# Kostis-S-Z/exploring_meta

Measured on AMD Instinct MI355X. Metric: tasks/sec, higher is better.
Workload: dtype f32

## Files before the change

### exploring_meta_amd/csrc/conv_b16.h

```cpp
#pragma once

#ifndef MI_CONV_B16_DEFAULT
#define MI_CONV_B16_DEFAULT 1
#endif

__device__ __forceinline__ void buf_st2_untracked(mi_u32x4 rsrc, unsigned off, float v0, float v1) {
  floatx2 v = {v0, v1};
  asm volatile("buffer_store_dwordx2 %0, %1, %2, 0 offen" : : "v"(v), "v"(off), "s"(rsrc) : "memory");
}
__device__ __forceinline__ floatx2 buf_ld8(mi_rsrc r, unsigned off) {
  return __builtin_bit_cast(floatx2, __builtin_amdgcn_raw_buffer_load_b64(r, off, 0, 0));
}
__device__ __forceinline__ int lane_mask_bit_rt(unsigned v, int bit) {
  int r;
  asm("v_bfe_i32 %0, %1, %2, 1" : "=v"(r) : "v"(v), "i"(bit));
  return r;
}
__device__ __forceinline__ float bf16_sub_v(float a, float b) {
  float r;
  asm volatile("v_sub_f32 %0, %1, %2" : "=v"(r) : "v"(a), "v"(b));
  return r;
}
#define MI_B16_MFMA(x, y, acc) __builtin_amdgcn_mfma_f32_16x16x32_bf16(MI_BF8(x), MI_BF8(y), acc, 0, 0, 0)

// ... 41 lines not shown
  {
    const unsigned total = gridDim.x * gridDim.y * gridDim.z;
    if ((total & 7u) == 0u) {
      const unsigned lin = (blockIdx.z * gridDim.y + blockIdx.y) * gridDim.x + blockIdx.x;
      const unsigned nl = (lin & 7u) * (total >> 3) + (lin >> 3);
      ct = (int)(nl % gridDim.z);
      bx = (int)((nl / gridDim.z) % gridDim.x);
      task = (int)(nl / (gridDim.z * gridDim.x));
    }
  }
  const int H = a.g.h, W = a.g.w;
  const int cbase = ct * 32;
  B16_ST(unsigned long long* stp = (blockIdx.x == 0 && blockIdx.y == 0 && blockIdx.z == 0 && (wave & 3) == 0 && lane == 0 && g_conv_stamps) ? g_conv_stamps + (wave >> 2) * 8 : nullptr;
         unsigned long long st_k = 0, st_epi = 0, st_n = 0, st_a = 0, st_b = 0, st_comb = 0; if (stp) stp[0] = __builtin_amdgcn_s_memtime();)

  {
    mi_u32x4* lw = reinterpret_cast<mi_u32x4*>(lds);
    constexpr int NIT = NU * 2 * 64, IPT = (NIT + NT - 1) / NT;
    floatx4 w0[IPT], w1[IPT];
#pragma unroll
    for (int q = 0; q < IPT; ++q) {
      const int it = tid + q * NT;
      const int ln = it & 63, grp = it >> 6;
      const int nb = grp & 1, u = grp >> 1;
      const int cc = u % NCC, tt = u / NCC, term = tt / 9, tap = tt - term * 9;
      const int k0 = cc * 32 + (ln >> 4) * 8, co = cbase + 2 * (ln & 15) + nb;
      const bool live = it < NIT;
      const float* wsrc = a.wt[live ? term : 0] + (size_t)task * a.wstride;
      if (MODE == 0) {
        const float* src = wsrc + ((size_t)(live ? tap : 0) * CI + k0) * CO + co;
#pragma unroll
// ... 379 lines not shown
```

### exploring_meta_amd/csrc/conv_mfma.hip

```cpp
#include "mi_common.h"
#include "kernels.h"
#include "bf16_split.h"
#include "fold.h"
#include <type_traits>

#ifdef MI_CONV_ABLATE_LOW
#define MI_LOW_PRODUCT(X)
#else
#define MI_LOW_PRODUCT(X) X
#endif
#ifdef MI_CONV_ABLATE_ROW
#define MI_ROW_KEPT(i) (hg_ddy(i) != 1)
#else
#define MI_ROW_KEPT(i) true
#endif
#define EPI_NONE 0
#define EPI_STATS 1
#define EPI_TSTATS 2
#define EPI_BRED 3

__device__ __forceinline__ void stats_block_reduce(double s, double q, double* ldsd, int lane, int wave, int nwaves,
                                                   double* partial_task, int co_total, int cbase, const FinArgs& fin, int task,
                                                   int bx = -1) {
  double* partial_blk = partial_task + (size_t)(bx < 0 ? (int)blockIdx.x : bx) * 2 * co_total;
// ... 233 lines not shown
  const int cbase = ct * 32;
  unsigned long long* cstamp = (blockIdx.x == 0 && blockIdx.y == 0 && blockIdx.z == 0) ? g_conv_stamps : nullptr;
  CV_STAMP(0);

  constexpr int NQ = BF ? 0 : NTERMS * 9 * CI * 32 / 4;
  float f16_sa[NTERMS], f16_sw[NTERMS], f16_inv = 1.f;
#pragma unroll
  for (int t = 0; t < NTERMS; ++t) { f16_sa[t] = 1.f; f16_sw[t] = 1.f; }
  unsigned f16_amax[NTERMS];
#pragma unroll
  for (int t = 0; t < NTERMS; ++t) f16_amax[t] = 0u;
  if constexpr (F16) {
#pragma unroll
    for (int t = 0; t < NTERMS; ++t) f16_amax[t] = mi_cell_fetch(a.amax[t], task);
  }
  if constexpr (BF) {
    mi_u32x4* l4 = reinterpret_cast<mi_u32x4*>(lds);
    constexpr int NIT = NSTEP * 2 * 64, IPT = (NIT + NT - 1) / NT;
    floatx4 w0[IPT], w1[IPT];
#pragma unroll
    for (int q = 0; q < IPT; ++q) {
      const int it = tid + q * NT;
      const int ln = it & 63, grp = it >> 6;
      const int jj = ln & 31, hb = ln >> 5, kb = grp & 1, stp = grp >> 1;
      const int cc = stp % NCC, tt = stp / NCC, term = tt / 9, tap = tt - term * 9;
      const int k0 = cc * 32 + hb * 16 + kb * 8;
      const bool live = it < NIT;
      const float* wsrc = a.wt[live ? term : 0] + (size_t)task * a.wstride;
      if (MODE == 0) {
        const float* src = wsrc + ((size_t)(live ? tap : 0) * CI + k0) * CO + cbase + jj;
#pragma unroll
// ... 850 lines not shown
    if (a.split_bf16) return launch_conv_s1_bf<CI, NTERMS, EPI, MODE, false>(st, a, grid);
  }
  const size_t lds = (size_t)NTERMS * 9 * CI * 32 * sizeof(float);
  auto k = conv3x3_s1_mfma_kernel<CI, NTERMS, EPI, MODE>;
  static unsigned attr_done = 0;
  if (hipError_t e = ensure_dynamic_lds(reinterpret_cast<const void*>(k), lds, &attr_done); e != hipSuccess) return e;
  hipLaunchKernelGGL(k, grid, dim3(ConvWaves<CI, NTERMS>::value * 64), lds, st, a);
  return hipGetLastError();
}

static bool conv_s1_ok(const ConvArgs& a) {
  return a.g.stride == 1 && a.g.co == a.g.ci && a.g.h == a.g.ho && a.g.w == a.g.wo && a.mpix < (1 << 24) &&
         (size_t)a.mpix * a.g.ci * 4 < (size_t)MI_OOB;
}

template <int CI, int NTERMS, int EPI>
static hipError_t launch_conv_ms(hipStream_t st, ConvArgs& a, dim3 grid, int mode, int stride) {
  if constexpr (EPI == EPI_BRED) {
    if (conv_s1_ok(a) && mode == 1) return launch_conv_s1<CI, NTERMS, EPI_BRED, 1>(st, a, grid);
    return hipErrorInvalidValue;
  } else {
    if (conv_s1_ok(a)) {
      if (mode == 0) return launch_conv_s1<CI, NTERMS, EPI, 0>(st, a, grid);
      if (EPI == EPI_NONE && mode == 1) return launch_conv_s1<CI, NTERMS, EPI_NONE, 1>(st, a, grid);
      return hipErrorInvalidValue;
    }
    if (mode == 0 && stride == 1) return launch_conv_t<CI, NTERMS, EPI, 0, 1>(st, a, grid);
    if (mode == 0 && stride == 2) return launch_conv_t<CI, NTERMS, EPI, 0, 2>(st, a, grid);
    if (EPI == EPI_NONE) {
      if (mode == 1 && stride == 1) return launch_conv_t<CI, NTERMS, EPI_NONE, 1, 1>(st, a, grid);
// ... 3 lines not shown
  }
}

hipError_t launch_conv3x3(hipStream_t st, ConvArgs a, int tasks, int nterms, int epi, int mode, int* blocks_per_task) {
  const int cot = a.g.co / 32;
  int ntiles, tpw;
  dim3 grid;
  a.split_bf16 = ((a.g.ci == 32 || (a.g.ci == 64 && nterms == 1)) && conv_s1_ok(a) && conv_split_bf16() &&
                  (epi == EPI_BRED ? mode == 1 : (mode == 0 || epi == EPI_NONE)) &&
                  ((g_conv_split_mask >> (((nterms - 1) * 2 + mode) * 4 + epi)) & 1u)) ? conv_operand_form() : 0;
  if (a.split_bf16 == 2 && (!a.amax[0] || (nterms == 2 && !a.amax[1]))) a.split_bf16 = 1;
  const int nw = ((a.split_bf16 == 2 && MI_F16_WIDE) || (nterms == 2 && a.g.ci == 32) || (a.split_bf16 && a.g.ci == 64)) ? 8 : 4;
  conv_grid(a.mpix, tasks, cot, nw, a.g.ci, nterms, ntiles, tpw, grid, a.split_bf16 ? 30 : 32, a.split_bf16 == 2 && MI_F16_WIDE && epi != EPI_TSTATS);
  a.ntiles = ntiles;
  a.tiles_per_wave = tpw;
  a.stagger = conv_stagger();
  if (blocks_per_task) *blocks_per_task = grid.x;
  if (a.g.co % 32 != 0) return hipErrorInvalidValue;
  const int s = a.g.stride;
  if (a.g.ci == 1 || a.g.ci == 3) {
    if (mode != 0 || nterms != 1) return hipErrorInvalidValue;
#define FIRST(CI0, E, S) hipLaunchKernelGGL((conv3x3_first_mfma_kernel<CI0, E, S>), grid, dim3(256), 0, st, a)
    if (a.g.ci == 3 && s == 1) { if (epi == EPI_STATS) FIRST(3, EPI_STATS, 1); else if (epi == EPI_TSTATS) FIRST(3, EPI_TSTATS, 1); else FIRST(3, EPI_NONE, 1); }
    else if (a.g.ci == 3 && s == 2) { if (epi == EPI_STATS) FIRST(3, EPI_STATS, 2); else if (epi == EPI_TSTATS) FIRST(3, EPI_TSTATS, 2); else FIRST(3, EPI_NONE, 2); }
    else if (a.g.ci == 1 && s == 1) { if (epi == EPI_STATS) FIRST(1, EPI_STATS, 1); else if (epi == EPI_TSTATS) FIRST(1, EPI_TSTATS, 1); else FIRST(1, EPI_NONE, 1); }
    else if (a.g.ci == 1 && s == 2) { if (epi == EPI_STATS) FIRST(1, EPI_STATS, 2); else if (epi == EPI_TSTATS) FIRST(1, EPI_TSTATS, 2); else FIRST(1, EPI_NONE, 2); }
    else return hipErrorInvalidValue;
#undef FIRST
    return hipGetLastError();
  }
// ... 1 lines not shown
  if (nterms == 1) {                                                                              \
    if (epi == EPI_NONE) return launch_conv_ms<CI, 1, EPI_NONE>(st, a, grid, mode, s);             \
    if (epi == EPI_STATS) return launch_conv_ms<CI, 1, EPI_STATS>(st, a, grid, mode, s);           \
    if (epi == EPI_BRED) return launch_conv_ms<CI, 1, EPI_BRED>(st, a, grid, mode, s);             \
    return launch_conv_ms<CI, 1, EPI_TSTATS>(st, a, grid, mode, s);                                \
  } else {                                                                                        \
    if (epi == EPI_NONE) return launch_conv_ms<CI, 2, EPI_NONE>(st, a, grid, mode, s);             \
    if (epi == EPI_TSTATS) return launch_conv_ms<CI, 2, EPI_TSTATS>(st, a, grid, mode, s);         \
    if (epi == EPI_BRED) return launch_conv_ms<CI, 2, EPI_BRED>(st, a, grid, mode, s);             \
    return hipErrorInvalidValue;                                                                  \
  }
  if (a.g.ci == 32) { DISPATCH(32) }
  if (a.g.ci == 64) { DISPATCH(64) }
#undef DISPATCH
  return hipErrorInvalidValue;
}

int wgrad_chunks(int mpix, int tasks) {
  int chunk = 1024;
  while (chunk > 32 && (long)ceil_div(mpix, chunk) * tasks < 2048) chunk >>= 1;
  return chunk;
}

static int rows_pick_rh(int w) {
  const int cand[4] = {7, 8, 5, 4};
  int best = 7, best_waste = 1 << 30;
  for (int i = 0; i < 4; ++i) {
    const int waste = ceil_div(w, cand[i]) * cand[i] - w;
    if (waste < best_waste) { best_waste = waste; best = cand[i]; }
  }
// ... 167 lines not shown
```

### exploring_meta_amd/csrc/engine.hip

```cpp
#include <string>
#include <vector>
#include <cstdio>
#include <cmath>
#include <cstring>
#include "mi_common.h"
#include "kernels.h"
#include "../../include/mi_maml.h"

#define EPI_NONE 0
#define EPI_STATS 1
#define EPI_TSTATS 2
#define EPI_BRED 3

static thread_local std::string g_err;

struct Layer {
  int ci, co, h, w, ho, wo, stride, pool, hp, wp;
  size_t off_gamma, off_beta, off_w, off_b;
};

static int gram_query_env() { static const int v = getenv("MI_GRAM_QUERY") ? atoi(getenv("MI_GRAM_QUERY")) : 2; return v; }
static bool fork_once_env() { static const bool v = getenv("MI_FORK_ONCE") && atoi(getenv("MI_FORK_ONCE")) != 0; return v; }
struct mi_engine {
  mi_model_desc d;
// ... 317 lines not shown
  float *xs, *xq;
  int32_t *ys, *yq;
  std::vector<ActSet> sup;
  ActSet qry;
  TanSet tan;
  double* bnpart;
  float* wgpart;
  float* wgpart_side;
  float* wgpart_l[8];
  double *gram_part, *gram_s;
  double *gram_q, *gram_part_q;
  int half = 0;
  float *tmp_loss, *tmp_acc;
  float* hscr;
  float* tail_wpart = nullptr; double* tail_bpart = nullptr; float* tail_scr = nullptr;
  unsigned* cells;
  int cell_cap, cell_used = 0, cell_T = 0;
  bool f16 = false;
  std::vector<std::pair<const void*, unsigned*>> cellmap;
  size_t bytes;
};

static void plan_actset(const mi_engine* e, Bump& b, ActSet& A, int T, int n, bool with_bwd) {
  const int nl = (int)e->L.size();
  A.zhm = nullptr;
  A.arg0 = nullptr;
  for (int l = 0; l < 8; ++l) A.zhl[l] = nullptr;
  for (int l = 0; l < nl; ++l) {
    const Layer& L = e->L[l];
    const size_t zs = (size_t)T * n * L.ho * L.wo * L.co, ps = (size_t)T * n * L.hp * L.wp * L.co;
// ... 4 lines not shown
    A.dp[l] = with_bwd ? b.take<float>(ps) : nullptr;
    if (fused && with_bwd && e->gram1) { A.zhm = b.take<float>(ps); A.arg0 = b.take<uint8_t>(ps); }
    A.zhl[l] = (!fused && with_bwd && l >= 1 && L.pool && dgrad_carries_reduce(e, l + 1)) ? b.take<float>(ps) : nullptr;
    A.mu[l] = b.take<float>((size_t)T * L.co);
    A.rstd[l] = b.take<float>((size_t)T * L.co);
  }
  if (e->d.head_mean_pool) {
    A.f = b.take<float>((size_t)T * n * e->feat);
    A.df = with_bwd ? b.take<float>((size_t)T * n * e->feat) : nullptr;
  } else {
    A.f = A.p[nl - 1];
    A.df = A.dp[nl - 1];
  }
  A.prob = b.take<float>((size_t)T * n * e->d.ways);
  A.dl = b.take<float>((size_t)T * n * e->d.ways);
}

static unsigned long long kernel_selection_key() {
  unsigned mask = 0;
  const unsigned form = (unsigned)mi_conv_get_split_bf16(&mask);
  return (unsigned long long)form + 4ull * (unsigned)conv_b16() + 16ull * (unsigned)block1_split_form() + 64ull * (unsigned)sparse_wgrad_split_form() + 128ull * (unsigned long long)mask;
}

static void make_plan(const mi_engine* e, void* ws, int T, int ns, int nq, int K, int second_order, Plan& pl) {
  Bump b{reinterpret_cast<char*>(ws), 0};
  const int nl = (int)e->L.size();
  const size_t TP = (size_t)T * e->PS;
  pl.theta = b.take<float>(TP * (K + 1));
  pl.g = b.take<float>(TP * (K > 0 ? K : 1));
  pl.lam = b.take<float>(TP);
// ... 72 lines not shown
      X.rdz[l] = (l == 0 && e->fuse1) ? nullptr : b.take<float>((size_t)T * ns * L.ho * L.wo * L.co);
    }
    X.dpd[0] = b.take<float>(pmax);
    X.dpd[1] = b.take<float>(pmax);
    if (e->d.head_mean_pool) {
      X.fd = b.take<float>((size_t)T * ns * e->feat);
      X.rdf = b.take<float>((size_t)T * ns * e->feat);
    } else {
      X.fd = nullptr;
      X.rdf = nullptr;
    }
  }
  pl.cell_cap = 8 + (K + 1) * 2 * nl + K * 4 * nl + 4 * nl;
  pl.cells = conv_operand_form() == 2 ? b.take<unsigned>((size_t)pl.cell_cap * T * MI_CELL_WORDS) : nullptr;
  pl.cell_T = T;
  pl.bytes = align_up(b.off, 256);
}

static int plan_begin(mi_engine* e, hipStream_t st, Plan& pl) {
  pl.f16 = conv_operand_form() == 2;
  pl.cell_used = 0;
  pl.cellmap.clear();
  if (pl.f16) HIPCHK(e, hipMemsetAsync(pl.cells, 0, (size_t)pl.cell_cap * pl.cell_T * MI_CELL_WORDS * sizeof(unsigned), st));
  return MI_OK;
}
static unsigned* cell_bind(mi_engine* e, Plan& pl, const void* tensor) {
  static const bool no_hooks = getenv("MI_F16_NO_PRODUCER_AMAX") && atoi(getenv("MI_F16_NO_PRODUCER_AMAX")) != 0;
  if (!pl.f16 || !tensor) return nullptr;
  for (auto it = pl.cellmap.begin(); it != pl.cellmap.end(); ++it)
    if (it->first == tensor) { pl.cellmap.erase(it); break; }
  if (no_hooks || pl.cell_used >= pl.cell_cap) return nullptr;
// ... 61 lines not shown
      !pl.tail_wpart)
    return false;
  const Layer& L = e->L[nl - 1];
  return tail_supported(n, L.ho, L.wo, L.co, L.pool, e->feat, e->d.ways);
}
static void tail_common(const mi_engine* e, const Plan& pl, TailArgs& ta) {
  ta.wpart = pl.tail_wpart; ta.bpart = pl.tail_bpart; ta.scr = pl.tail_scr; ta.counter = e->counters; ta.stamps = e->tail_stamps;
}
extern "C" int mi_debug_tail_stamps(mi_engine* e, unsigned long long* buf) {
  if (!e) return MI_ERR_ARG;
  e->tail_stamps = buf;
  return MI_OK;
}

static int trunk_forward(mi_engine* e, hipStream_t st, Plan& pl, ActSet& A, const float* x0, int n, int T, const float* theta,
                         const double* gram = nullptr, bool stats_ready = false, bool skip_last_bn = false) {
  const int nl = (int)e->L.size();
  const size_t P = e->PS;
  for (int l = 0; l < nl; ++l) {
    const Layer& L = e->L[l];
    if (l == 0 && e->fuse1) {
      B1Args ba = b1_args(e, pl, A, x0, n, theta);
      int blk = 0;
      if (gram && stats_ready) {
      } else if (gram) {
        LAUNCH(e, st, OP_GRAM_STATS, 0, launch_gram_stats(st, gram, T, L.ci, L.co, theta + L.off_w, P, nullptr, 0, 1.0 / ((double)n * L.ho * L.wo), 0, A.mu[0], A.rstd[0], nullptr, nullptr));
      } else {
        ba.fin = fin_of(e, T, 1.0 / ((double)n * L.ho * L.wo), FIN_STATS, A.mu[0], L.co, A.rstd[0], L.co);
        LAUNCH(e, st, OP_CONV_FWD, 0, launch_block1(st, ba, T, L.ci, B1_STATS, &blk));
        if (!ba.fin.counter)
          LAUNCH(e, st, OP_BN_FINALIZE, 0, launch_bn_finalize(st, pl.bnpart, blk, T, L.co, 1.0 / ((double)n * L.ho * L.wo), FIN_STATS, A.mu[0], L.co, A.rstd[0], L.co));
        ba.fin = FinArgs{};
      }
// ... 4 lines not shown
      ba.fwd_fp32 = (gram && A.arg0) ? 0 : 1;
      LAUNCH(e, st, OP_BN_FWD, 0, launch_block1(st, ba, T, L.ci, B1_FWD, nullptr));
      continue;
    }
    ConvArgs ca{};
    ca.in[0] = l == 0 ? x0 : A.p[l - 1];
    ca.wt[0] = theta + L.off_w;
    ca.wstride = P;
    ca.out = A.z[l];
    ca.partial = pl.bnpart;
    ca.g = geom(L, n);
    ca.mpix = n * L.ho * L.wo;
    int blk = 0;
    ca.fin = fin_of(e, T, 1.0 / (double)ca.mpix, FIN_STATS, A.mu[l], L.co, A.rstd[l], L.co);
    if (l >= 1) CELL(ca.in[0], (size_t)n * L.h * L.w * L.ci, ca.amax[0]);
    LAUNCH(e, st, OP_CONV_FWD, l, launch_conv3x3(st, ca, T, 1, EPI_STATS, 0, &blk));
    if (!ca.fin.counter)
      LAUNCH(e, st, OP_BN_FINALIZE, l, launch_bn_finalize(st, pl.bnpart, blk, T, L.co, 1.0 / (double)ca.mpix, FIN_STATS, A.mu[l], L.co, A.rstd[l], L.co));
    if (skip_last_bn && l == nl - 1) break;
    BnArgs ba{};
    ba.z = A.z[l]; ba.mu = A.mu[l]; ba.rstd = A.rstd[l];
    ba.gamma = theta + L.off_gamma; ba.beta = theta + L.off_beta; ba.pstride = P;
    ba.out = A.p[l];
    ba.zh_out = A.zhl[l];
    ba.n = n; ba.ho = L.ho; ba.wo = L.wo; ba.c = L.co;
    ba.amax_out = cell_bind(e, pl, ba.out);
    LAUNCH(e, st, OP_BN_FWD, l, launch_bn_fwd(st, ba, T, L.pool));
  }
  return MI_OK;
}

static const float* zh_at_argmax(const mi_engine* e, const ActSet& A, int lower) {
  return (lower == 0 && e->fuse1) ? A.zhm : A.zhl[lower];
}

static void adv_add_seg(AdvanceArgs* adv, size_t off, int nelem, const float* partial, int nchunks) {
  AdvanceSeg& sg = adv->seg[adv->nseg++];
  sg.off = (unsigned)off; sg.nelem = (unsigned)nelem; sg.partial = partial; sg.nchunks = nchunks;
}
static int trunk_backward(mi_engine* e, hipStream_t st, Plan& pl, ActSet& A, const float* x0, int n, int T, const float* theta,
                          float* g, const double* gram = nullptr, AdvanceArgs* adv = nullptr, bool last_bn_done = false) {
  const int nl = (int)e->L.size();
  const size_t P = e->PS;
  bool forked = false, red_done[9] = {false, false, false, false, false, false, false, false, false};
  WgradArgs held[9]; int held_l[9], nheld = 0;
  for (int l = nl - 1; l >= 0; --l) {
    const Layer& L = e->L[l];
    const int mpix = n * L.ho * L.wo;
    const bool b1red_done = red_done[0];
    if (l == 0 && e->fuse1) {
      B1Args b1 = b1_args(e, pl, A, x0, n, theta);
      b1.dp = A.dp[0];
      int blk = 0;
      const FinArgs fin = fin_of(e, T, 1.0, FIN_SUMS, g + L.off_gamma, P, g + L.off_beta, P);
      if (b1red_done) {
      } else if (A.zhm) {
        PoolRedArgs pr{A.p[0], A.zhm, nullptr, A.dp[0], nullptr, pl.bnpart, n * L.hp * L.wp, L.co, fin};
        LAUNCH(e, st, OP_BN_BWD_REDUCE, 0, launch_pooled_reduce(st, pr, T, 0, &blk));
// ... 71 lines not shown
    } else {
      hipStream_t ws = l > 0 ? side_fork(e, st, pl.half) : st;
      if (ws != st) forked = true;
      const int rc = issue_wgrad(ws, wa, l);
      if (rc) return rc;
    }
    if (l > 0) {
      ConvArgs ca{};
      ca.in[0] = A.dz[l];
      ca.wt[0] = theta + L.off_w;
      ca.wstride = P;
      ca.out = A.dp[l - 1];
      ca.amax[0] = wa.amax_dz[0];
      ca.g = geom_dgrad(L, n);
      ca.mpix = n * L.h * L.w;
      const float* zh_lo = dgrad_carries_reduce(e, l) ? zh_at_argmax(e, A, l - 1) : nullptr;
      if (zh_lo) {
        const Layer& L0 = e->L[l - 1];
        ca.bp = A.p[l - 1]; ca.bzh = zh_lo; ca.partial = pl.bnpart;
        ca.barg = (l - 1 == 0 && e->fuse1 && e->bred_arg) ? A.arg0 : nullptr;
        ca.fin = fin_of(e, T, 1.0, FIN_SUMS, g + L0.off_gamma, P, g + L0.off_beta, P);
        int blk0 = 0;
        LAUNCH(e, st, OP_DGRAD, l, launch_conv3x3(st, ca, T, 1, EPI_BRED, 1, &blk0));
        if (!ca.fin.counter)
          LAUNCH(e, st, OP_BN_FINALIZE, l - 1, launch_bn_finalize(st, pl.bnpart, blk0, T, L0.co, 1.0, FIN_SUMS, g + L0.off_gamma, P, g + L0.off_beta, P));
        red_done[l - 1] = true;
      } else {
        LAUNCH(e, st, OP_DGRAD, l, launch_conv3x3(st, ca, T, 1, EPI_NONE, 1, nullptr));
      }
    }
  }
  return side_join(e, st, pl.half, forked);
}

static void head_scratch(const mi_engine* e, HeadArgs& ha, float* hscr, int T, int n) {
  ha.rdl = hscr;
  ha.rowloss = hscr + (size_t)T * n * e->d.ways;
  ha.rowhit = ha.rowloss + (size_t)T * n;
}

static int head_pass(mi_engine* e, hipStream_t st, float* hscr, const float* f, const int32_t* y, int n, int T, const float* theta,
                     float* g, float* loss, float* acc, float* logits, float* prob, float* dl, float* df, bool with_grad) {
  const size_t P = e->PS;
  HeadArgs ha{};
  ha.f = f;
  ha.wl = theta + e->off_wl; ha.bl = theta + e->off_bl; ha.pstride = P;
// ... 23 lines not shown
  return MI_OK;
}

struct ExportPause {
  mi_engine* e; float* buf;
  explicit ExportPause(mi_engine* e_) : e(e_), buf(e_ ? e_->bn_export : nullptr) { if (e) e->bn_export = nullptr; }
  ~ExportPause() { if (e) e->bn_export = buf; }
};

static int pass_fwd_bwd(mi_engine* e, hipStream_t st, Plan& pl, ActSet& A, const float* x0, const int32_t* y, int n, int T,
                        const float* theta, float* g, float* loss, float* acc, float* logits, bool with_grad,
                        const double* gram = nullptr, AdvanceArgs* adv = nullptr, bool stats_ready = false, int Tb = -1) {
  const int nl = (int)e->L.size();
  if (Tb < 0) Tb = T;
  const bool fused_last = fused_last_ok(e, pl, n, T);
  int rc = trunk_forward(e, st, pl, A, x0, n, T, theta, gram, stats_ready, fused_last);
  if (rc) return rc;
  rc = export_bn_stats(e, st, A, T);
  if (rc) return rc;
  if (e->d.head_mean_pool) HIPCHK(e, launch_spatial_mean(st, A.p[nl - 1], A.f, T * n, e->head_hw, e->head_c));
  if (with_grad && !adv) HIPCHK(e, hipMemsetAsync(g, 0, (size_t)T * e->PS * sizeof(float), st));
  if (fused_last) {
    const Layer& L = e->L[nl - 1];
    const size_t P = e->PS;
    TailArgs ta{};
    BnArgs& ba = ta.bn;
    ba.z = A.z[nl - 1]; ba.mu = A.mu[nl - 1]; ba.rstd = A.rstd[nl - 1];
    ba.gamma = theta + L.off_gamma; ba.beta = theta + L.off_beta; ba.pstride = P;
    ba.dp = A.dp[nl - 1]; ba.out = A.dz[nl - 1];
    ba.n = n; ba.ho = L.ho; ba.wo = L.wo; ba.c = L.co;
    ba.inv_m = 1.f / (float)(n * L.ho * L.wo);
// ... 15 lines not shown
  }
  rc = head_pass(e, st, pl.hscr, A.f, y, n, T, theta, g, loss, acc, logits, A.prob, A.dl, A.df, with_grad);
  if (rc || !with_grad || Tb == 0) return rc;
  if (e->d.head_mean_pool) HIPCHK(e, launch_spatial_mean_bwd(st, A.df, A.dp[nl - 1], Tb * n, e->head_hw, e->head_c));
  return trunk_backward(e, st, pl, A, x0, n, Tb, theta, g, gram, adv);
}

static int pass_hvp(mi_engine* e, hipStream_t st, Plan& pl, ActSet& A, const float* x0, int n, int T, const float* theta,
                    const float* g, const float* v, float* hv, const double* gram = nullptr, const float* dl_fixed = nullptr,
                    float* ld_out = nullptr, AdvanceArgs* adv = nullptr, bool stats_ready = false) {
  const int nl = (int)e->L.size();
  const size_t P = e->PS;
  TanSet& X = pl.tan;
  const bool fused_last = !dl_fixed && !ld_out && fused_last_ok(e, pl, n, T);
  if (!adv) HIPCHK(e, hipMemsetAsync(hv, 0, (size_t)T * P * sizeof(float), st));
  for (int l = 0; l < nl; ++l) {
    const Layer& L = e->L[l];
    const int mpix = n * L.ho * L.wo;
    if (l == 0 && e->fuse1) {
      B1Args b1 = b1_args(e, pl, A, x0, n, theta);
      b1.wd = v + L.off_w; b1.vstride = P;
      int blk = 0;
      if (gram && stats_ready) {
      } else if (gram) {
        LAUNCH(e, st, OP_GRAM_STATS, 0, launch_gram_stats(st, gram, T, L.ci, L.co, theta + L.off_w, P, v + L.off_w, P, 1.0 / (double)mpix, 1, X.m1[0], X.m2[0], A.mu[0], A.rstd[0]));
      } else {
        b1.fin = fin_of(e, T, 1.0 / (double)mpix, FIN_TSTATS, X.m1[0], L.co, X.m2[0], L.co);
        LAUNCH(e, st, OP_TAN_CONV, 0, launch_block1(st, b1, T, L.ci, B1_TSTATS, &blk));
        if (!b1.fin.counter)
          LAUNCH(e, st, OP_BN_FINALIZE, 0, launch_bn_finalize(st, pl.bnpart, blk, T, L.co, 1.0 / (double)mpix, FIN_TSTATS, X.m1[0], L.co, X.m2[0], L.co));
// ... 16 lines not shown
    ConvArgs ca{};
    ca.in[0] = l == 0 ? x0 : A.p[l - 1];
    ca.wt[0] = v + L.off_w;
    if (l > 0) { ca.in[1] = X.pd[l - 1]; ca.wt[1] = theta + L.off_w; }
    ca.wstride = P;
    ca.out = X.zd[l];
    ca.z = A.z[l]; ca.mu = A.mu[l]; ca.rstd = A.rstd[l];
    ca.partial = pl.bnpart;
    ca.g = geom(L, n);
    ca.mpix = mpix;
    int blk = 0;
    ca.fin = fin_of(e, T, 1.0 / (double)mpix, FIN_TSTATS, X.m1[l], L.co, X.m2[l], L.co);
    if (l >= 1) {
      CELL(ca.in[0], (size_t)n * L.h * L.w * L.ci, ca.amax[0]);
      CELL(ca.in[1], (size_t)n * L.h * L.w * L.ci, ca.amax[1]);
    }
    LAUNCH(e, st, OP_TAN_CONV, l, launch_conv3x3(st, ca, T, l > 0 ? 2 : 1, EPI_TSTATS, 0, &blk));
    if (!ca.fin.counter)
      LAUNCH(e, st, OP_BN_FINALIZE, l, launch_bn_finalize(st, pl.bnpart, blk, T, L.co, 1.0 / (double)mpix, FIN_TSTATS, X.m1[l], L.co, X.m2[l], L.co));
    if (fused_last && l == nl - 1) break;
    BnArgs ba{};
    ba.z = A.z[l]; ba.zd = X.zd[l]; ba.mu = A.mu[l]; ba.rstd = A.rstd[l]; ba.m1 = X.m1[l]; ba.m2 = X.m2[l];
    ba.gamma = theta + L.off_gamma; ba.beta = theta + L.off_beta; ba.pstride = P;
    ba.gammad = v + L.off_gamma; ba.betad = v + L.off_beta; ba.vstride = P;
    ba.out = X.pd[l];
    ba.zh_out = A.zhl[l] ? X.zhdl[l] : nullptr;
    ba.n = n; ba.ho = L.ho; ba.wo = L.wo; ba.c = L.co;
    ba.amax_out = cell_bind(e, pl, ba.out);
    LAUNCH(e, st, OP_BN_TAN_FWD, l, launch_bn_tan_fwd(st, ba, T, L.pool));
  }
// ... 136 lines not shown
    } else {
      hipStream_t ws = l > 0 ? side_fork(e, st, pl.half) : st;
      if (ws != st) forked = true;
      const int rc = issue_wgrad(ws, wa, l);
      if (rc) return rc;
    }
    if (l > 0) {
      ConvArgs ca{};
      ca.in[0] = X.rdz[l]; ca.wt[0] = theta + L.off_w;
      ca.in[1] = A.dz[l]; ca.wt[1] = v + L.off_w;
      ca.amax[0] = wa.amax_dz[0]; ca.amax[1] = wa.amax_dz[1];
      ca.wstride = P;
      ca.out = X.dpd[cur ^ 1];
      ca.g = geom_dgrad(L, n);
      ca.mpix = n * L.h * L.w;
      const float* zh_lo = dgrad_carries_reduce(e, l) ? zh_at_argmax(e, A, l - 1) : nullptr;
      const float* zhd_lo = (l - 1 == 0 && e->fuse1) ? X.zhdm : X.zhdl[l - 1];
      if (zh_lo && zhd_lo) {
        const Layer& L0 = e->L[l - 1];
        ca.bp = A.p[l - 1]; ca.bzh = zh_lo; ca.bzhd = zhd_lo; ca.bdp = A.dp[l - 1]; ca.partial = pl.bnpart;
        ca.barg = (l - 1 == 0 && e->fuse1 && e->bred_arg) ? A.arg0 : nullptr;
        ca.fin = fin_of(e, T, 1.0, FIN_SUMS, hv + L0.off_gamma, P, hv + L0.off_beta, P);
        int blk0 = 0;
        LAUNCH(e, st, OP_TAN_DGRAD, l, launch_conv3x3(st, ca, T, 2, EPI_BRED, 1, &blk0));
        if (!ca.fin.counter)
          LAUNCH(e, st, OP_BN_FINALIZE, l - 1, launch_bn_finalize(st, pl.bnpart, blk0, T, L0.co, 1.0, FIN_SUMS, hv + L0.off_gamma, P, hv + L0.off_beta, P));
        red_done[l - 1] = true;
      } else {
        LAUNCH(e, st, OP_TAN_DGRAD, l, launch_conv3x3(st, ca, T, 2, EPI_NONE, 1, nullptr));
      }
      cur ^= 1;
    }
  }
  return side_join(e, st, pl.half, forked);
}

static AdvanceArgs advance_base(const mi_engine* e, float* g) {
  AdvanceArgs a{};
  a.g = g; a.gstride = e->PS; a.ostride = e->PS; a.n = (unsigned)e->PS;
  a.nzero = e->nzero;
  for (int z = 0; z < e->nzero; ++z) { a.zoff[z] = e->zoff[z]; a.zlen[z] = e->zlen[z]; }
  a.off_w1 = (unsigned)e->L[0].off_w;
  a.ci = (e->L[0].ci == 1 || e->L[0].ci == 3) ? e->L[0].ci : 0;
  a.co = e->L[0].co;
  a.counter = e->counters;
  return a;
}

// ... 157 lines not shown
      w = (size_t)T * bpt * 9 * L.ci * L.co;
    }
    if (w > wgp) wgp = w;
  }
  ap.scratch.bnpart = b.take<double>(bnp);
  ap.scratch.wgpart = b.take<float>(wgp);
  ap.scratch.wgpart_side = b.take<float>(wgp);
  ap.scratch.gram_part = ap.scratch.gram_s = nullptr;
  ap.scratch.cell_cap = 8 + 4 * (int)e->L.size();
  ap.scratch.cells = conv_operand_form() == 2 ? b.take<unsigned>((size_t)ap.scratch.cell_cap * T * MI_CELL_WORDS) : nullptr;
  ap.scratch.cell_T = T;
  if (e->fuse1 && e->gram1 && gram_supported(e->L[0].w, e->L[0].ci)) {
    ap.scratch.gram_part = b.take<double>(gram_partial_doubles(T, 2 * n, e->L[0].h, e->L[0].ci));
    ap.scratch.gram_s = b.take<double>(gram_doubles(T, e->L[0].ci));
  }
  ap.bytes = align_up(b.off, 256);
}

extern "C" int mi_anil_workspace_bytes(const mi_engine* e, int tasks, int ways, int shots, int adapt_steps, size_t* bytes) {
  if (!e || !bytes || tasks < 1 || ways < 1 || shots < 1 || adapt_steps < 0) return MI_ERR_ARG;
  AnilPlan ap;
  make_anil_plan(e, nullptr, tasks, ways * shots, adapt_steps, ap);
  *bytes = ap.bytes;
  return MI_OK;
}

static int meta_batch_anil_impl(mi_engine* e, void* stream, const float* theta, const float* data, const int64_t* labels,
                                int tasks, int ways, int shots, int adapt_steps, float inner_lr, int second_order,
                                int with_grad, float* loss_out, float* acc_out, float* meta_grad_out, float* logits_out,
                                void* workspace, size_t workspace_bytes) {
// ... 496 lines not shown
```

### exploring_meta_amd/csrc/kernels.h

```cpp
#pragma once
#include "mi_common.h"
#include "finalize.h"

struct ConvArgs {
  const float* in[2];
  const float* wt[2];
  size_t wstride;
  float* out;
  const float* z;
  const float* mu;
  const float* rstd;
  double* partial;
  FinArgs fin;
  const float *bp, *bzh, *bzhd, *bdp;
  const uint8_t* barg;
  ConvGeom g;
  int mpix;
  int ntiles, tiles_per_wave;
  int split_bf16;
  int stagger;
  const unsigned* amax[2];
};

struct WgradArgs {
  const float* x[2];
  const float* dz[2];
  float* partial;
  ConvGeom g;
  int mpix, chunk_pix, nchunks, nterms;
  const unsigned* amax_x[2]; const unsigned* amax_dz[2];
  int form;
};

struct BnArgs {
  const float* z;
  const float* zd;
  const float* mu;
// ... 22 lines not shown
  const float* zhd;
  const float* dp;
  const float* dpd;
  double* partial;
  int rows, c;
  FinArgs fin;
};
int pooled_reduce_blocks(int rows, int c, int tasks);
hipError_t launch_pooled_reduce(hipStream_t st, const PoolRedArgs& a, int tasks, int tangent, int* nblk);

int conv_operand_form();
int conv_b16();
int block1_split_form();
int sparse_wgrad_split_form();
hipError_t launch_conv3x3(hipStream_t st, ConvArgs a, int tasks, int nterms, int epi, int mode, int* blocks_per_task);
hipError_t launch_wgrad3x3(hipStream_t st, WgradArgs a, int tasks, int nterms, int* nchunks_out);
hipError_t launch_wgrad_reduce(hipStream_t st, const float* partial, int nchunks, int nelem, int tasks, float* out, size_t ostride);
size_t wgrad_partial_floats(const ConvGeom& g, int tasks);
int conv_max_blocks_per_task(const ConvGeom& g);
int conv_tiles_per_wave(int mpix, int tasks, int cot);

int bn_blocks_per_task(int n, int ho, int wo, int c, int pool, int tasks);
hipError_t launch_bn_finalize(hipStream_t st, const double* partial, int nblk, int tasks, int c, double inv_m, int mode,
                              float* out0, size_t stride0, float* out1, size_t stride1);
hipError_t launch_bn_fwd(hipStream_t st, const BnArgs& a, int tasks, int pool);
hipError_t launch_bn_bwd_reduce(hipStream_t st, const BnArgs& a, int tasks, int pool, int* nblk);
hipError_t launch_bn_bwd_apply(hipStream_t st, const BnArgs& a, int tasks, int pool);
hipError_t launch_bn_tan_fwd(hipStream_t st, const BnArgs& a, int tasks, int pool);
hipError_t launch_bn_tan_bwd_reduce(hipStream_t st, const BnArgs& a, int tasks, int pool, int* nblk);
hipError_t launch_bn_tan_bwd_apply(hipStream_t st, const BnArgs& a, int tasks, int pool);
// ... 156 lines not shown
```

Before: 1933.

## Pre-split conv weights into bf16 planes once per pass and load them directly

Adds a presplit kernel that converts each layer's f32 weights into hi/mid/lo bf16 planes, already laid out in the LDS image order that the b16 and MFMA conv kernels expect. The result is stored in workspace buffers and bound to the conv launches for forward, dgrad and tangent passes. The intent is to stop every conv block from reloading strided f32 weights and redoing the bf16 split, so each block only copies a contiguous plane image into LDS. In exchange it adds an extra launch per pass, more workspace memory, and bookkeeping that matches planes to weight vectors and task counts.

```diff
diff --git a/exploring_meta_amd/csrc/conv_b16.h b/exploring_meta_amd/csrc/conv_b16.h
--- a/exploring_meta_amd/csrc/conv_b16.h
+++ b/exploring_meta_amd/csrc/conv_b16.h
@@ -79,7 +79,23 @@
   B16_ST(unsigned long long* stp = (blockIdx.x == 0 && blockIdx.y == 0 && blockIdx.z == 0 && (wave & 3) == 0 && lane == 0 && g_conv_stamps) ? g_conv_stamps + (wave >> 2) * 8 : nullptr;
          unsigned long long st_k = 0, st_epi = 0, st_n = 0, st_a = 0, st_b = 0, st_comb = 0; if (stp) stp[0] = __builtin_amdgcn_s_memtime();)
 
-  {
+  if (a.wp[0]) {
+    mi_u32x4* lw = reinterpret_cast<mi_u32x4*>(lds);
+    constexpr int PER = 9 * NCC * 3 * 2 * 64, NPI = NTERMS * PER, CPT = (NPI + NT - 1) / NT;
+    mi_u32x4 pv[CPT];
+#pragma unroll
+    for (int q = 0; q < CPT; ++q) {
+      const int it = tid + q * NT;
+      const int term = (NTERMS == 2 && it >= PER) ? 1 : 0;
+      const int r = it < NPI ? it - term * PER : 0;
+      pv[q] = reinterpret_cast<const mi_u32x4*>(a.wp[term])[((size_t)task * gridDim.z + ct) * PER + r];
+    }
+#pragma unroll
+    for (int q = 0; q < CPT; ++q) {
+      const int it = tid + q * NT;
+      if (it < NPI) lw[it] = pv[q];
+    }
+  } else {
     mi_u32x4* lw = reinterpret_cast<mi_u32x4*>(lds);
     constexpr int NIT = NU * 2 * 64, IPT = (NIT + NT - 1) / NT;
     floatx4 w0[IPT], w1[IPT];
diff --git a/exploring_meta_amd/csrc/conv_mfma.hip b/exploring_meta_amd/csrc/conv_mfma.hip
--- a/exploring_meta_amd/csrc/conv_mfma.hip
+++ b/exploring_meta_amd/csrc/conv_mfma.hip
@@ -271,7 +271,28 @@
 #pragma unroll
     for (int t = 0; t < NTERMS; ++t) f16_amax[t] = mi_cell_fetch(a.amax[t], task);
   }
-  if constexpr (BF) {
+  bool planes_given = false;
+  if constexpr (BF && !F16) {
+    if (a.wp[0]) {
+      planes_given = true;
+      mi_u32x4* l4 = reinterpret_cast<mi_u32x4*>(lds);
+      constexpr int PER = 9 * NCC * 2 * 3 * 64, NPI = NTERMS * PER, CPT = (NPI + NT - 1) / NT;
+      mi_u32x4 pv[CPT];
+#pragma unroll
+      for (int q = 0; q < CPT; ++q) {
+        const int it = tid + q * NT;
+        const int term = (NTERMS == 2 && it >= PER) ? 1 : 0;
+        const int r = it < NPI ? it - term * PER : 0;
+        pv[q] = reinterpret_cast<const mi_u32x4*>(a.wp[term])[((size_t)task * gridDim.z + ct) * PER + r];
+      }
+#pragma unroll
+      for (int q = 0; q < CPT; ++q) {
+        const int it = tid + q * NT;
+        if (it < NPI) l4[it] = pv[q];
+      }
+    }
+  }
+  if constexpr (BF) if (!planes_given) {
     mi_u32x4* l4 = reinterpret_cast<mi_u32x4*>(lds);
     constexpr int NIT = NSTEP * 2 * 64, IPT = (NIT + NT - 1) / NT;
     floatx4 w0[IPT], w1[IPT];
@@ -1152,6 +1173,50 @@
          (size_t)a.mpix * a.g.ci * 4 < (size_t)MI_OOB;
 }
 
+__global__ __launch_bounds__(256) void presplit_kernel(PresplitArgs a) {
+  const PresplitJob jb = a.job[blockIdx.z];
+  const int C = a.c, NCC = C >> 5, cot = C >> 5;
+  const int nit1 = 9 * NCC * 2 * 64;
+  const int it = blockIdx.x * 256 + threadIdx.x, task = blockIdx.y;
+  if (it >= cot * nit1) return;
+  const int ct = it / nit1, r = it - ct * nit1;
+  const int ln = r & 63, grp = r >> 6, u = grp >> 1;
+  const int cc = u % NCC, tap = u / NCC;
+  int k0, co;
+  if (jb.img == PLANE_IMG_B16) { k0 = cc * 32 + (ln >> 4) * 8; co = ct * 32 + 2 * (ln & 15) + (grp & 1); }
+  else { k0 = cc * 32 + (ln >> 5) * 16 + (grp & 1) * 8; co = ct * 32 + (ln & 31); }
+  const float* wsrc = jb.w + (size_t)task * a.wstride;
+  floatx4 w0, w1;
+  if (jb.mode == 0) {
+    const float* src = wsrc + ((size_t)tap * C + k0) * C + co;
+#pragma unroll
+    for (int i = 0; i < 4; ++i) { w0[i] = src[(size_t)i * C]; w1[i] = src[(size_t)(i + 4) * C]; }
+  } else {
+    const float* src = wsrc + ((size_t)tap * C + co) * C + k0;
+    w0 = *reinterpret_cast<const floatx4*>(src);
+    w1 = *reinterpret_cast<const floatx4*>(src + 4);
+  }
+  Bf16Planes pw;
+  bf16_split8(w0, w1, pw);
+  mi_u32x4* dst = reinterpret_cast<mi_u32x4*>(jb.out) + ((size_t)task * cot + ct) * (size_t)(nit1 * 3);
+  const int i0 = jb.img == PLANE_IMG_B16 ? ((u * 3) * 2 + (grp & 1)) * 64 + ln : (grp * 3) * 64 + ln;
+  const int ps = jb.img == PLANE_IMG_B16 ? 128 : 64;
+  dst[i0] = mi_u32x4{pw.h[0], pw.h[1], pw.h[2], pw.h[3]};
+  dst[i0 + ps] = mi_u32x4{pw.m[0], pw.m[1], pw.m[2], pw.m[3]};
+  dst[i0 + 2 * ps] = mi_u32x4{pw.l[0], pw.l[1], pw.l[2], pw.l[3]};
+}
+size_t conv_plane_bytes(int c, int tasks) { return (size_t)tasks * (c / 32) * 9 * (c / 32) * 2 * 64 * 3 * 16; }
+hipError_t launch_presplit(hipStream_t st, const PresplitArgs& a, int tasks) {
+  if (a.njobs < 1) return hipSuccess;
+  if (a.njobs > 28 || (a.c != 32 && a.c != 64) || tasks < 1 || tasks > 65535) return hipErrorInvalidValue;
+  for (int j = 0; j < a.njobs; ++j)
+    if (!a.job[j].w || !a.job[j].out || (a.job[j].img != PLANE_IMG_B16 && a.job[j].img != PLANE_IMG_MFMA)) return hipErrorInvalidValue;
+  const int items = (a.c / 32) * 9 * (a.c / 32) * 2 * 64;
+  hipLaunchKernelGGL(presplit_kernel, dim3(ceil_div(items, 256), tasks, a.njobs), dim3(256), 0, st, a);
+  return hipGetLastError();
+}
+bool conv_presplit() { static const bool v = !(getenv("MI_PRESPLIT") && atoi(getenv("MI_PRESPLIT")) == 0); return v; }
+
 template <int CI, int NTERMS, int EPI>
 static hipError_t launch_conv_ms(hipStream_t st, ConvArgs& a, dim3 grid, int mode, int stride) {
   if constexpr (EPI == EPI_BRED) {
@@ -1185,6 +1250,9 @@
   conv_grid(a.mpix, tasks, cot, nw, a.g.ci, nterms, ntiles, tpw, grid, a.split_bf16 ? 30 : 32, a.split_bf16 == 2 && MI_F16_WIDE && epi != EPI_TSTATS);
   a.ntiles = ntiles;
   a.tiles_per_wave = tpw;
+  if (!conv_presplit() || a.split_bf16 != 1 || !a.wp[0] || (nterms == 2 && !a.wp[1]) ||
+      a.wp_img != (conv_b16_for(a) ? PLANE_IMG_B16 : PLANE_IMG_MFMA))
+    a.wp[0] = a.wp[1] = nullptr;
   a.stagger = conv_stagger();
   if (blocks_per_task) *blocks_per_task = grid.x;
   if (a.g.co % 32 != 0) return hipErrorInvalidValue;
@@ -1216,6 +1284,19 @@
   if (a.g.ci == 64) { DISPATCH(64) }
 #undef DISPATCH
   return hipErrorInvalidValue;
+}
+
+int conv_plane_image(const ConvGeom& g, int mpix, int tasks, int nterms, int mode) {
+  ConvArgs a{};
+  a.g = g; a.mpix = mpix;
+  if (!conv_presplit() || !((g.ci == 32 || (g.ci == 64 && nterms == 1)) && conv_s1_ok(a) && conv_split_bf16()) || conv_operand_form() != 1)
+    return PLANE_IMG_NONE;
+  const int nw = ((nterms == 2 && g.ci == 32) || g.ci == 64) ? 8 : 4;
+  int ntiles, tpw;
+  dim3 grid;
+  conv_grid(mpix, tasks, g.co / 32, nw, g.ci, nterms, ntiles, tpw, grid, 30, false);
+  a.tiles_per_wave = tpw;
+  return conv_b16_for(a) ? PLANE_IMG_B16 : PLANE_IMG_MFMA;
 }
 
 int wgrad_chunks(int mpix, int tasks) {
diff --git a/exploring_meta_amd/csrc/engine.hip b/exploring_meta_amd/csrc/engine.hip
--- a/exploring_meta_amd/csrc/engine.hip
+++ b/exploring_meta_amd/csrc/engine.hip
@@ -355,6 +355,8 @@
   float *tmp_loss, *tmp_acc;
   float* hscr;
   float* tail_wpart = nullptr; double* tail_bpart = nullptr; float* tail_scr = nullptr;
+  struct PlaneSlot { const float* vec = nullptr; void* buf[8][2] = {}; int img[8][2] = {}; } pw[2];
+  int pw_bwd_tasks = 0;
   unsigned* cells;
   int cell_cap, cell_used = 0, cell_T = 0;
   bool f16 = false;
@@ -389,6 +391,18 @@
   }
   A.prob = b.take<float>((size_t)T * n * e->d.ways);
   A.dl = b.take<float>((size_t)T * n * e->d.ways);
+}
+
+static bool plane_layer(const mi_engine* e, int l) {
+  const Layer& L = e->L[l];
+  return l >= 1 && L.stride == 1 && L.ci == L.co && (L.ci == 32 || L.ci == 64);
+}
+static void plan_planes(const mi_engine* e, Bump& b, Plan& pl, int T, bool with_direction) {
+  if (!conv_presplit() || conv_operand_form() != 1) return;
+  for (int s = 0; s < (with_direction ? 2 : 1); ++s)
+    for (int l = 0; l < (int)e->L.size(); ++l)
+      if (plane_layer(e, l))
+        for (int m = 0; m < 2; ++m) pl.pw[s].buf[l][m] = b.take<char>(conv_plane_bytes(e->L[l].ci, T));
 }
 
 static unsigned long long kernel_selection_key() {
@@ -491,7 +505,52 @@
   pl.cell_cap = 8 + (K + 1) * 2 * nl + K * 4 * nl + 4 * nl;
   pl.cells = conv_operand_form() == 2 ? b.take<unsigned>((size_t)pl.cell_cap * T * MI_CELL_WORDS) : nullptr;
   pl.cell_T = T;
+  plan_planes(e, b, pl, T, second_order && K > 0);
   pl.bytes = align_up(b.off, 256);
+}
+
+static void planes_jobs(const mi_engine* e, Plan& pl, int slot, const float* vec, int n, int fwd_tasks, int bwd_tasks, int nterms, PresplitArgs& pa) {
+  Plan::PlaneSlot& S = pl.pw[slot];
+  S.vec = vec;
+  for (int l = 0; l < (int)e->L.size(); ++l) {
+    const Layer& L = e->L[l];
+    for (int m = 0; m < 2; ++m) {
+      const int tasks = m == 0 ? fwd_tasks : bwd_tasks;
+      S.img[l][m] = PLANE_IMG_NONE;
+      if (!S.buf[l][m] || tasks < 1) continue;
+      const int img = conv_plane_image(m == 0 ? geom(L, n) : geom_dgrad(L, n), m == 0 ? n * L.ho * L.wo : n * L.h * L.w, tasks, nterms, m);
+      if (img == PLANE_IMG_NONE || pa.njobs >= 28) continue;
+      S.img[l][m] = img;
+      pa.job[pa.njobs++] = PresplitJob{vec + L.off_w, S.buf[l][m], m, img};
+    }
+  }
+}
+static const void* planes_get(const Plan& pl, const float* vec, int l, int mode, int* img) {
+  for (int s = 0; s < 2; ++s)
+    if (pl.pw[s].vec == vec && pl.pw[s].img[l][mode] > 0) { *img = pl.pw[s].img[l][mode]; return pl.pw[s].buf[l][mode]; }
+  return nullptr;
+}
+static void planes_release(Plan& pl) {
+  pl.pw_bwd_tasks = 0;
+  for (int s = 0; s < 2; ++s) { pl.pw[s].vec = nullptr; for (int l = 0; l < 8; ++l) pl.pw[s].img[l][0] = pl.pw[s].img[l][1] = PLANE_IMG_NONE; }
+}
+static void planes_release(Plan& pl);
+static int planes_produce(mi_engine* e, hipStream_t st, Plan& pl, int n, const float* v0, const float* v1, int fwd_tasks, int bwd_tasks, int nterms) {
+  planes_release(pl);
+  PresplitArgs pa{};
+  pa.c = e->d.hidden; pa.wstride = e->PS;
+  planes_jobs(e, pl, 0, v0, n, fwd_tasks, bwd_tasks, nterms, pa);
+  if (v1) planes_jobs(e, pl, 1, v1, n, fwd_tasks, bwd_tasks, nterms, pa);
+  pl.pw_bwd_tasks = bwd_tasks;
+  if (pa.njobs) LAUNCH(e, st, OP_MISC, 6, launch_presplit(st, pa, fwd_tasks > bwd_tasks ? fwd_tasks : bwd_tasks));
+  return MI_OK;
+}
+static void planes_bind(const Plan& pl, ConvArgs& ca, const float* v0, const float* v1, int l, int mode) {
+  int i0 = 0, i1 = 0;
+  const void* p0 = planes_get(pl, v0, l, mode, &i0);
+  const void* p1 = v1 ? planes_get(pl, v1, l, mode, &i1) : nullptr;
+  if (!p0 || (v1 && (!p1 || i1 != i0))) return;
+  ca.wp[0] = p0; ca.wp[1] = p1; ca.wp_img = i0;
 }
 
 static int plan_begin(mi_engine* e, hipStream_t st, Plan& pl) {
@@ -583,9 +642,10 @@
 }
 
 static int trunk_forward(mi_engine* e, hipStream_t st, Plan& pl, ActSet& A, const float* x0, int n, int T, const float* theta,
-                         const double* gram = nullptr, bool stats_ready = false, bool skip_last_bn = false) {
+                         const double* gram = nullptr, bool stats_ready = false, bool skip_last_bn = false, int bwd_tasks = 0) {
   const int nl = (int)e->L.size();
   const size_t P = e->PS;
+  { const int prc = planes_produce(e, st, pl, n, theta, nullptr, T, bwd_tasks, 1); if (prc) return prc; }
   for (int l = 0; l < nl; ++l) {
     const Layer& L = e->L[l];
     if (l == 0 && e->fuse1) {
@@ -620,6 +680,7 @@
     int blk = 0;
     ca.fin = fin_of(e, T, 1.0 / (double)ca.mpix, FIN_STATS, A.mu[l], L.co, A.rstd[l], L.co);
     if (l >= 1) CELL(ca.in[0], (size_t)n * L.h * L.w * L.ci, ca.amax[0]);
+    planes_bind(pl, ca, theta, nullptr, l, 0);
     LAUNCH(e, st, OP_CONV_FWD, l, launch_conv3x3(st, ca, T, 1, EPI_STATS, 0, &blk));
     if (!ca.fin.counter)
       LAUNCH(e, st, OP_BN_FINALIZE, l, launch_bn_finalize(st, pl.bnpart, blk, T, L.co, 1.0 / (double)ca.mpix, FIN_STATS, A.mu[l], L.co, A.rstd[l], L.co));
@@ -648,6 +709,7 @@
                           float* g, const double* gram = nullptr, AdvanceArgs* adv = nullptr, bool last_bn_done = false) {
   const int nl = (int)e->L.size();
   const size_t P = e->PS;
+  if (!(pl.pw[0].vec == theta && pl.pw_bwd_tasks == T)) { const int prc = planes_produce(e, st, pl, n, theta, nullptr, 0, T, 1); if (prc) return prc; }
   bool forked = false, red_done[9] = {false, false, false, false, false, false, false, false, false};
   WgradArgs held[9]; int held_l[9], nheld = 0;
   for (int l = nl - 1; l >= 0; --l) {
@@ -749,6 +811,7 @@
       ca.amax[0] = wa.amax_dz[0];
       ca.g = geom_dgrad(L, n);
       ca.mpix = n * L.h * L.w;
+      planes_bind(pl, ca, theta, nullptr, l, 1);
       const float* zh_lo = dgrad_carries_reduce(e, l) ? zh_at_argmax(e, A, l - 1) : nullptr;
       if (zh_lo) {
         const Layer& L0 = e->L[l - 1];
@@ -765,6 +828,7 @@
       }
     }
   }
+  planes_release(pl);
   return side_join(e, st, pl.half, forked);
 }
 
@@ -818,7 +882,7 @@
   const int nl = (int)e->L.size();
   if (Tb < 0) Tb = T;
   const bool fused_last = fused_last_ok(e, pl, n, T);
-  int rc = trunk_forward(e, st, pl, A, x0, n, T, theta, gram, stats_ready, fused_last);
+  int rc = trunk_forward(e, st, pl, A, x0, n, T, theta, gram, stats_ready, fused_last, with_grad ? Tb : 0);
   if (rc) return rc;
   rc = export_bn_stats(e, st, A, T);
   if (rc) return rc;
@@ -864,6 +928,7 @@
   TanSet& X = pl.tan;
   const bool fused_last = !dl_fixed && !ld_out && fused_last_ok(e, pl, n, T);
   if (!adv) HIPCHK(e, hipMemsetAsync(hv, 0, (size_t)T * P * sizeof(float), st));
+  { const int prc = planes_produce(e, st, pl, n, theta, v, T, T, 2); if (prc) return prc; }
   for (int l = 0; l < nl; ++l) {
     const Layer& L = e->L[l];
     const int mpix = n * L.ho * L.wo;
@@ -910,6 +975,7 @@
     if (l >= 1) {
       CELL(ca.in[0], (size_t)n * L.h * L.w * L.ci, ca.amax[0]);
       CELL(ca.in[1], (size_t)n * L.h * L.w * L.ci, ca.amax[1]);
+      planes_bind(pl, ca, v, theta, l, 0);
     }
     LAUNCH(e, st, OP_TAN_CONV, l, launch_conv3x3(st, ca, T, l > 0 ? 2 : 1, EPI_TSTATS, 0, &blk));
     if (!ca.fin.counter)
@@ -1076,6 +1142,7 @@
       ca.out = X.dpd[cur ^ 1];
       ca.g = geom_dgrad(L, n);
       ca.mpix = n * L.h * L.w;
+      planes_bind(pl, ca, theta, v, l, 1);
       const float* zh_lo = dgrad_carries_reduce(e, l) ? zh_at_argmax(e, A, l - 1) : nullptr;
       const float* zhd_lo = (l - 1 == 0 && e->fuse1) ? X.zhdm : X.zhdl[l - 1];
       if (zh_lo && zhd_lo) {
@@ -1094,6 +1161,7 @@
       cur ^= 1;
     }
   }
+  planes_release(pl);
   return side_join(e, st, pl.half, forked);
 }
 
@@ -1281,6 +1349,7 @@
     ap.scratch.gram_part = b.take<double>(gram_partial_doubles(T, 2 * n, e->L[0].h, e->L[0].ci));
     ap.scratch.gram_s = b.take<double>(gram_doubles(T, e->L[0].ci));
   }
+  plan_planes(e, b, ap.scratch, T, false);
   ap.bytes = align_up(b.off, 256);
 }
 
diff --git a/exploring_meta_amd/csrc/kernels.h b/exploring_meta_amd/csrc/kernels.h
--- a/exploring_meta_amd/csrc/kernels.h
+++ b/exploring_meta_amd/csrc/kernels.h
@@ -20,7 +20,12 @@
   int split_bf16;
   int stagger;
   const unsigned* amax[2];
-};
+  const void* wp[2];
+  int wp_img;
+};
+enum { PLANE_IMG_NONE = 0, PLANE_IMG_B16 = 1, PLANE_IMG_MFMA = 2 };
+struct PresplitJob { const float* w; void* out; int mode, img; };
+struct PresplitArgs { PresplitJob job[28]; int njobs; int c; size_t wstride; };
 
 struct WgradArgs {
   const float* x[2];
@@ -73,6 +78,10 @@
 int block1_split_form();
 int sparse_wgrad_split_form();
 hipError_t launch_conv3x3(hipStream_t st, ConvArgs a, int tasks, int nterms, int epi, int mode, int* blocks_per_task);
+bool conv_presplit();
+int conv_plane_image(const ConvGeom& g, int mpix, int tasks, int nterms, int mode);
+size_t conv_plane_bytes(int c, int tasks);
+hipError_t launch_presplit(hipStream_t st, const PresplitArgs& a, int tasks);
 hipError_t launch_wgrad3x3(hipStream_t st, WgradArgs a, int tasks, int nterms, int* nchunks_out);
 hipError_t launch_wgrad_reduce(hipStream_t st, const float* partial, int nchunks, int nelem, int tasks, float* out, size_t ostride);
 size_t wgrad_partial_floats(const ConvGeom& g, int tasks);
```

Result: no change. 1922, median of 2 (-0.6%).
